# mkofler96/DeepSDF

Measured on AMD Instinct MI355X. Metric: SDF point-samples/sec per training step (8x512 decoder, 16384 pts), higher is better.
Workload: dtype f32; 1 GPU; configs[1]: 64 synthetic sphere-SDF scenes, latent_dim=256, 8x512 decoder + layer-4 skip, weight-norm, dropout 0.2, 16384 pts/step (64 scenes x 256 samples), fp32; headline_config=True, parallelism=dp1

## Files before the change

### deepsdf_amd/csrc/dsdf_api.hip

```cpp
#include "../../include/dsdf.h"

#include <hip/hip_runtime.h>
#include <math.h>
#include <stdarg.h>
#include <stdio.h>
#include <string.h>

#include <stdlib.h>

#include <algorithm>
#include <atomic>
#ifdef DSDF_LAB
#include <vector>
#endif

#include "dwstream.hpp"
#include "sample.hpp"
#include "fused.hpp"
#include "fused_bf16x8.hpp"
#include "gemm.hpp"
#include "kernels.hpp"
#include "mcubes.hpp"
#include "meshsdf.hpp"
#include "msgrid.hpp"
// ... 534 lines not shown
struct FamilyKernels {
  FwdKernel fwd; int fwd_block;
  FwdKernel fwd_act;
  BwdKernel bwd;
  FwdBwdKernel fwd_bwd;
  DwKernel dw;
  int block;
};
const FamilyKernels KERNELS[FAM_COUNT] = {
     {nullptr, 0, nullptr, nullptr, nullptr, nullptr, 0},
     {fused_forward_kernel, 256, fused_forward_kernel, fused_backward_kernel, fused_fwd_bwd_kernel, dw_stream_kernel, 256},
     {fused_forward_split_kernel, 256, fused_forward_split_kernel, fused_backward_split_kernel, fused_fwd_bwd_split_kernel,
                          dw_stream_split_kernel, 256},
     {fused_forward_bf16x8_kernel, F8_THREADS, fused_forward_bf16_kernel, fused_backward_kernel, fused_fwd_bf16_bwd_kernel,
                          dw_stream_kernel, 256},
     {fused_forward_bf16x8_kernel, F8_THREADS, fused_forward_bf16_kernel, fused_backward_split_kernel,
                          fused_fwd_bf16_bwd_split_kernel, dw_stream_split_kernel, 256},
     {fused_forward_h32_kernel, 256, fused_forward_h32_kernel, nullptr, fused_fwd_bwd_h32_kernel, dw_stream_kernel, 256},
     {fused_forward_n128_kernel, 256, fused_forward_n128_kernel, fused_backward_kernel, fused_fwd_bwd_n128_kernel,
                          dw_stream_kernel, 256},
     {nullptr, 0, nullptr, nullptr, fused_fwd_bwd_w32_kernel, dw_stream_kernel, 64},
     {nullptr, 0, nullptr, nullptr, fused_fwd_bwd_w32x2_kernel, dw_stream_kernel, 64},
};

bool fused_eligible(const DsdfNet* net) {
  if (net_variant(net)) return false;
  if (net->in_dim[0] > FMAXW) return false;
  for (int l = 0; l < net->n_layers - 1; ++l)
    if (net->in_dim[l] > FMAXW || net->out_dim[l] > FMAXW) return false;
  return net->in_dim[net->n_layers - 1] <= FMAXW;
}

Path pick_path(const DsdfNet* net, int64_t n, Entry entry, const Switches& sw) {
  Path p{FAM_LAYERED, FROWS, false, false};
  if (sw.no_fused || !fused_eligible(net)) return p;
  p.fused = true;
  p.merged = entry == ENTRY_TRAIN && !sw.no_merge;
  if (net->fwd_bf16 || net->gemm_split) {
    p.family = !net->fwd_bf16 ? FAM_SPLIT : (net->gemm_split ? FAM_BF16_SPLIT : FAM_BF16);
    return p;
  }
  int wmax = 0;
  for (int l = 0; l < net->n_layers; ++l) {
    wmax = std::max(wmax, net->in_dim[l]);
    if (l < net->n_layers - 1) wmax = std::max(wmax, net->out_dim[l]);
  }
  const bool narrow = !sw.no_narrow && wmax <= 128;
  p.family = narrow ? FAM_N128 : FAM_FP32;
  const bool rows32 = entry == ENTRY_INFER || p.merged;
  if (!rows32 || sw.frows64 || n <= 0) return p;
  if (p.merged && narrow && !sw.no_w32 && (wmax <= FWW || (wmax <= FWW2 && !sw.no_w32x2))) {
    p.family = wmax <= FWW ? FAM_W32 : FAM_W32X2;
    p.frows = 32;
  } else if (n <= 32ll * (chip_waves() / 4)) {
    p.family = FAM_H32;
    p.frows = 32;
  }
  return p;
}

struct Drop { bool on; uint32_t thr; float scale; };
Drop drop_of(const DsdfNet* net, int layer, int training) {
  Drop d{training && ((net->dropout_mask >> layer) & 1) && net->dropout_p > 0.f, 0u, 1.0f};
  if (d.on) {
    d.thr = (uint32_t)std::min(lround((double)net->dropout_p * 65536.0), 65535l);
    d.scale = 1.0f / (1.0f - net->dropout_p);
  }
  return d;
}
float mask_scale_of(const DsdfNet* net, int layer, int training) { return drop_of(net, layer, training).scale; }

struct Call {
  const DsdfNet* net;
  Switches sw;
  Path path;
  Plan P;
  DsdfParamLayout L;
  Packed pk;
  void* ws;
  const float* packed;
  const float* params;
  int64_t n;
  hipStream_t st;
  int training;
  const uint32_t* keys;
  uint32_t row_offset;
  template <typename T>
  T* at(size_t off) const { return reinterpret_cast<T*>(static_cast<char*>(ws) + off); }
};

int run_gather(const Call& c, const float* table, const DsdfBatch* b, const float* input, int64_t ld_in) {
  GatherArgs g;
  memset(&g, 0, sizeof(g));
  g.table = table; g.L = c.net->latent_size; g.G = c.net->geom_dim;
  if (b) { g.xyz = b->xyz; g.seg_scene = b->seg_scene; g.seg_offset = b->seg_offset; g.R = (int)b->n_segments; }
  g.input = input; g.ld_in = ld_in; g.n = (int)c.n;
  const int W0 = c.net->latent_size + c.net->geom_dim;
  const bool drop = c.net->latent_dropout && c.training && c.keys != nullptr && c.net->latent_size > 0;
  if (drop) { g.drop_key = c.keys[LATENT_DROPOUT_KEY]; g.drop_thr = latent_drop_thr(); g.drop_scale = 1.0f / (1.0f - LATENT_DROPOUT_P); g.row_offset = c.row_offset; }
  g.ndst = 0;
  g.dst[g.ndst++] = GatherDst{c.at<float>(c.P.in_off[0]), c.P.ld_in[0], 0, 0, W0, drop ? 1 : 0};
  for (int l = 1; l < c.net->n_layers; ++l) {
    if ((c.net->skip_mask >> l) & 1) g.dst[g.ndst++] = GatherDst{c.at<float>(c.P.in_off[l]), c.P.ld_in[l], c.net->out_dim[l - 1], 0, W0, 0};
    else if (c.net->xyz_in_all) g.dst[g.ndst++] = GatherDst{c.at<float>(c.P.in_off[l]), c.P.ld_in[l], c.net->out_dim[l - 1], c.net->latent_size, c.net->geom_dim, 0};
  }
  hipLaunchKernelGGL(gather_concat_kernel, dim3((unsigned)((c.n + 3) / 4)), dim3(256), 0, c.st, g);
  LAUNCH_OK("gather_concat_kernel");
  return 0;
}

#ifdef DSDF_LAB
struct LabStamps { const char* env; size_t bytes; bool zero; unsigned long long* dev; };
struct LabScope {
  LabStamps& s;
  LabScope(LabStamps& site, hipStream_t st) : s(site) {
    if (!s.dev && getenv(s.env)) (void)hipMalloc(&s.dev, s.bytes);
    if (s.dev && s.zero) (void)hipMemsetAsync(s.dev, 0, s.bytes, st);
  }
  ~LabScope() {
    if (!s.dev || !getenv(s.env)) return;
    (void)hipDeviceSynchronize();
    std::vector<unsigned long long> h(s.bytes / 8);
    (void)hipMemcpy(h.data(), s.dev, s.bytes, hipMemcpyDeviceToHost);
    FILE* f = fopen(getenv(s.env), "wb");
    if (f) { fwrite(h.data(), 1, s.bytes, f); fclose(f); }
  }
};
#endif

struct HoistRenorm { float max_norm; float* dlat; long long nzero; };
int run_hoist(const Call& c, const float* table, const DsdfBatch* b, FusedSeg* seg, const HoistRenorm* renorm = nullptr) {
  if (c.net->latent_size < 1 || c.net->latent_size > HOIST_MAXL)
    return fail(DSDF_E_INVALID, "segment mode needs 1 <= latent_size <= %d (got %d)", HOIST_MAXL, c.net->latent_size);
  const int ks = skip_layer(c.net);
  HoistArgs h;
  memset(&h, 0, sizeof(h));
  memset(seg, 0, sizeof(*seg));
  h.nh = ks > 0 ? 2 : 1;
  h.W[0] = c.packed + c.pk.w_off[0]; h.ldw[0] = c.pk.ldw[0]; h.c0[0] = 0; h.out[0] = c.net->out_dim[0];
  seg->h[0].layer = 0; seg->h[0].wx = h.W[0] + c.net->latent_size; seg->h[0].ldw = c.pk.ldw[0];
  seg->h[1].layer = -1;
  if (ks > 0) {
    h.W[1] = c.packed + c.pk.w_off[ks]; h.ldw[1] = c.pk.ldw[ks]; h.c0[1] = c.net->out_dim[ks - 1]; h.out[1] = c.net->out_dim[ks];
    seg->h[1].layer = ks; seg->h[1].wx = h.W[1] + h.c0[1] + c.net->latent_size; seg->h[1].ldw = c.pk.ldw[ks];
  }
  h.L = c.net->latent_size; h.seg_scene = b->seg_scene; h.table = table; h.R = (int)b->n_segments;
  h.U = c.at<float>(c.P.hoistU_off); h.ldu = c.P.ldu;
  h.bf16 = c.net->fwd_bf16 ? 1 : 0;
  if (renorm != nullptr) {
    h.max_norm = renorm->max_norm; h.zr = c.at<float>(c.P.zr_off);
    h.dlat = renorm->nzero > 0 ? renorm->dlat : nullptr; h.nzero = renorm->nzero;
  }
  const int rows = h.out[0] + (ks > 0 ? h.out[1] : 0);
  const dim3 hgrid((unsigned)((rows + 3) / 4), (unsigned)((h.R + HOIST_SC - 1) / HOIST_SC));
  switch ((h.L + 63) >> 6) {
    case 1: hipLaunchKernelGGL(seg_hoist_kernel<1>, hgrid, dim3(256), 0, c.st, h); break;
    case 2: hipLaunchKernelGGL(seg_hoist_kernel<2>, hgrid, dim3(256), 0, c.st, h); break;
    case 3: case 4: hipLaunchKernelGGL(seg_hoist_kernel<4>, hgrid, dim3(256), 0, c.st, h); break;
    default: hipLaunchKernelGGL(seg_hoist_kernel<8>, hgrid, dim3(256), 0, c.st, h); break;
  }
  LAUNCH_OK("seg_hoist_kernel");
  seg->wg_per_seg = (int)(b->seg_len / c.P.frows);
  seg->xyz = b->xyz; seg->G = c.net->geom_dim; seg->U = h.U; seg->ldu = h.ldu;
  return 0;
}

int run_fused_forward(const Call& c, bool store_act, float* y_out, float* u_out, const FusedSeg* seg = nullptr,
                      FusedFwdArgs* defer = nullptr) {
  const int last = c.net->n_layers - 1;
  FusedFwdArgs a;
  memset(&a, 0, sizeof(a));
  a.n_hidden = last; a.N = (int)c.n; a.W0 = c.net->in_dim[0];
  a.x0 = c.at<float>(c.P.in_off[0]); a.ldx0 = c.P.ld_in[0];
  a.row_offset = c.row_offset;
  for (int l = 0; l < last; ++l) {
    FusedLayer& y = a.ly[l];
    y.wf = c.net->fwd_bf16 ? c.packed + c.pk.wfb_off[l] : (c.net->gemm_split ? c.packed + c.pk.ws_off[l] : c.packed + c.pk.wf_off[l]);
    y.wplane = (int)(c.pk.ws_plane[l] * 2);
    y.wf32 = c.packed + c.pk.wf_off[l];
    y.bias = c.params + c.L.bias_off[l];
    y.out = store_act ? c.at<float>(c.P.in_off[l + 1]) : nullptr;
    y.ld_out = c.P.ld_in[l + 1];
    y.in = c.net->in_dim[l]; y.out_dim = c.net->out_dim[l]; y.U = c.pk.uf[l];
    const Drop drop = drop_of(c.net, l, c.training);
    if (drop.on) { y.drop_thr = drop.thr; y.drop_key = c.keys[l]; y.drop_scale = drop.scale; }
    y.x0_col = ((c.net->skip_mask >> (l + 1)) & 1) ? c.net->out_dim[l] : -1;
    y.maskbits = store_act ? c.at<uint32_t>(c.P.mask_off[l]) : nullptr;
    if (seg != nullptr) {
      y.x0_col = -1;
      if (l == 0) y.in = 0;
      else if ((c.net->skip_mask >> l) & 1) y.in = c.net->out_dim[l - 1];
    }
  }
  if (seg != nullptr) a.seg = *seg;
  a.w_last = c.packed + c.pk.w_off[last]; a.b_last = c.params + c.L.bias_off[last]; a.in_last = c.net->in_dim[last];
  a.use_tanh = c.net->use_tanh; a.y_out = y_out; a.u_out = u_out;
  if (defer != nullptr) {
    a.ly[last - 1].out = nullptr;
    *defer = a;
    return 0;
  }
  double wmac = 0;
  for (int l = 0; l < last; ++l) wmac += (double)c.net->in_dim[l] * c.net->out_dim[l];
  ProfScope ps(DSDF_PROF_FUSED_FWD, 2.0 * (double)c.n * wmac, c.st);
#ifdef DSDF_LAB
  static LabStamps stamps{"DSDF_LAB_DBG", 8192 * 64 * 8, false, nullptr};
  LabScope lab(stamps, c.st);
  a.dbg = stamps.dev;
#endif
  const FamilyKernels& k = KERNELS[c.path.family];
  const FwdKernel kernel = store_act ? k.fwd_act : k.fwd;
  if (kernel == nullptr) return fail(DSDF_E_LAUNCH, "internal: kernel family %d has no forward of its own", (int)c.path.family);
  const dim3 grid((unsigned)((c.n + c.P.frows - 1) / c.P.frows));
  hipLaunchKernelGGL(kernel, grid, dim3(store_act ? k.block : k.fwd_block), 0, c.st, a);
  LAUNCH_OK("fused_forward_kernel");
  return 0;
}

int run_hidden_forward(const Call& c, bool save_ln = true) {
  for (int l = 0; l < c.net->n_layers - 1; ++l) {
    NtArgs a;
    memset(&a, 0, sizeof(a));
    a.A = c.at<float>(c.P.in_off[l]); a.lda = c.P.ld_in[l];
    a.B = c.packed + c.pk.w_off[l]; a.ldb = c.pk.ldw[l];
    a.C = c.at<float>(c.P.in_off[l + 1]); a.ldc = c.P.ld_in[l + 1];
    a.M = (int)c.n; a.N = c.net->out_dim[l]; a.K = c.net->in_dim[l];
    a.bias = c.params + c.L.bias_off[l];
    a.relu = 1;
    const Drop drop = drop_of(c.net, l, c.training);
    if (ln_applied(c.net, l)) {
      a.C = c.at<float>(c.P.lnx_off[l]);
      TRY(launch_nt<EPI_PLAIN>(a, c.st));
      LnFwdArgs f;
      memset(&f, 0, sizeof(f));
      f.y = a.C; f.ldy = a.ldc; f.gamma = c.params + c.L.ln_w_off[l]; f.beta = c.params + c.L.ln_b_off[l];
      f.out = c.at<float>(c.P.in_off[l + 1]); f.ldo = c.P.ld_in[l + 1]; f.n = (int)c.n; f.width = c.net->out_dim[l];
      f.save = save_ln ? 1 : 0; f.rstd = save_ln ? c.at<float>(c.P.lnr_off[l]) : nullptr;
      if (drop.on) { f.drop_thr = drop.thr; f.drop_key = c.keys[l]; f.drop_scale = drop.scale; f.row_offset = c.row_offset; }
      hipLaunchKernelGGL(ln_fwd_kernel, dim3((unsigned)((c.n + 3) / 4)), dim3(256), 0, c.st, f);
      LAUNCH_OK("ln_fwd_kernel");
      continue;
    }
    if (drop.on) { a.drop_thr = drop.thr; a.drop_key = c.keys[l]; a.drop_scale = drop.scale; a.row_offset = c.row_offset; }
    TRY(launch_nt<EPI_FWD>(a, c.st));
  }
  return 0;
}

struct FuseAdam { const DsdfAdamCfg* cfg; float* params; float* exp_avg; float* exp_avg_sq; float* packed; bool used; };

struct FinSrc { const float* slabs; int nsplit; long long slab; int ldc; const float* colsum; int npart; int ldcs; };
struct GradSink { float* grads; int accumulate; const FuseAdam* fz; };
FinArgs fin_args(const Call& c, int l, const FinSrc& src, const GradSink& to) {
  FinArgs f;
  memset(&f, 0, sizeof(f));
  f.slabs = src.slabs; f.nsplit = src.nsplit; f.slab = src.slab; f.ldc = src.ldc;
  f.colsum = src.colsum; f.npart = src.npart; f.ldcs = src.ldcs;
  f.g = c.L.g_off[l] >= 0 ? c.params + c.L.g_off[l] : nullptr;
  f.v = c.params + c.L.v_off[l];
  f.dg = c.L.g_off[l] >= 0 ? to.grads + c.L.g_off[l] : nullptr;
  f.dv = to.grads + c.L.v_off[l];
  f.db = to.grads + c.L.bias_off[l];
  f.out = c.net->out_dim[l]; f.in = c.net->in_dim[l]; f.accumulate = to.accumulate;
  if (to.fz != nullptr) {
    const DsdfAdamCfg* ad = to.fz->cfg;
    const double bc1 = 1.0 - pow((double)ad->beta1, (double)ad->step), bc2 = 1.0 - pow((double)ad->beta2, (double)ad->step);
    f.adam = 1;
    f.pb = to.fz->params + c.L.bias_off[l]; f.mb = to.fz->exp_avg + c.L.bias_off[l]; f.sb = to.fz->exp_avg_sq + c.L.bias_off[l];
    f.pv = to.fz->params + c.L.v_off[l];    f.mv = to.fz->exp_avg + c.L.v_off[l];    f.sv = to.fz->exp_avg_sq + c.L.v_off[l];
    if (c.L.g_off[l] >= 0) { f.pg = to.fz->params + c.L.g_off[l]; f.mg = to.fz->exp_avg + c.L.g_off[l]; f.sg = to.fz->exp_avg_sq + c.L.g_off[l]; }
    int r0 = 0;
    for (int q = 0; q < l; ++q) r0 += c.net->out_dim[q];
    f.scale_out = to.fz->packed + c.pk.scale_off + r0;
    f.omb1 = 1.0f - ad->beta1; f.b2 = ad->beta2; f.omb2 = 1.0f - ad->beta2;
    f.step_size = (float)((double)ad->lr_decoder / bc1); f.bc2_sqrt = (float)sqrt(bc2); f.eps = ad->eps;
  }
  return f;
}

int add_dz_to_input(const Call& c, bool used_dzB, float* d_input, int64_t ld_din) {
  const long long tot = (long long)c.n * c.P.W0;
  hipLaunchKernelGGL(add2_kernel, dim3((unsigned)((tot + 255) / 256)), dim3(256), 0, c.st, c.at<float>(c.P.dzA_off), c.P.ldz,
                     used_dzB ? c.at<float>(c.P.dzB_off) : nullptr, c.P.ldz, d_input, (long long)ld_din, (int)c.n, c.P.W0);
  LAUNCH_OK("add2_kernel");
  return 0;
}

LastArgs last_args(const Call& c, bool backward = false) {
  const int last = c.net->n_layers - 1;
  LastArgs a;
  memset(&a, 0, sizeof(a));
  a.a = c.at<float>(c.P.in_off[last]); a.lda = c.P.ld_in[last]; a.in = c.net->in_dim[last];
  a.w = c.packed + c.pk.w_off[last]; a.b = c.params + c.L.bias_off[last]; a.n = (int)c.n; a.use_tanh = c.net->use_tanh;
  if (!backward) return a;
  a.dp_prev = c.at<float>(c.P.dp_off[0]);
  a.lddp = c.P.ld_dp; a.mask_scale = mask_scale_of(c.net, last - 1, c.training);
  a.part_dw = c.at<float>(c.P.part_off); a.ld_part = c.P.ld_part;
  a.part_colsum = c.at<float>(c.P.part_off) + c.P.ld_in[last];
  a.part_db = c.at<float>(c.P.partdb_off); a.part_loss = c.at<float>(c.P.partloss_off);
  a.n_act = c.net->out_dim[last - 1];
  return a;
}

int run_backward(const Call& c, const GradSink& to, int ncols_dz, bool* used_dzB, bool want_dw, bool* xyz_acc = nullptr) {
  const int last = c.net->n_layers - 1;
  if (want_dw) {
    const int w = c.P.ld_part;
// ... 2469 lines not shown
```

### deepsdf_amd/csrc/kernels.hpp

```cpp
#pragma once
#include "common.hpp"

namespace dsdf {

constexpr int FSEG_MAXW = 512;

__global__ void latent_renorm_kernel(float* __restrict__ table, int L, const int64_t* __restrict__ seg_scene,
                                     int R, float max_norm, float* __restrict__ dlat, long long nzero) {
  if (dlat != nullptr)
    for (long long i = ((long long)blockIdx.x * blockDim.x + threadIdx.x) * 4; i < nzero; i += (long long)gridDim.x * blockDim.x * 4) {
      if (i + 3 < nzero) *reinterpret_cast<float4*>(dlat + i) = make_float4(0.f, 0.f, 0.f, 0.f);
      else for (long long q = i; q < nzero; ++q) dlat[q] = 0.f;
    }
  const int r = blockIdx.x * (blockDim.x >> 6) + (threadIdx.x >> 6);
  const int lane = threadIdx.x & 63;
  if (r >= R || max_norm <= 0.f) return;
  const int64_t j = seg_scene[r];
  int dup = 0;
  for (int q = lane; q < r; q += 64) dup |= (seg_scene[q] == j);
  if (__any(dup)) return;
  float* row = table + (size_t)j * L;
  float ss = 0.f;
  for (int c = lane; c < L; c += 64) { const float v = row[c]; ss += v * v; }
  ss = wave_sum(ss);
  const float nu = sqrtf(ss);
  if (nu > max_norm) {
    const float s = max_norm / (nu + 1e-7f);
    for (int c = lane; c < L; c += 64) row[c] *= s;
  }
}

struct GatherDst { float* ptr; int ld; int col0; int src0; int ncols; int drop; };
struct GatherArgs {
  const float* table; int L; const float* xyz; int G;
  const int64_t* seg_scene; const int64_t* seg_offset; int R;
  const float* input; long long ld_in;
  uint32_t drop_key, drop_thr; float drop_scale; uint32_t row_offset;
  int n; int ndst; GatherDst dst[DSDF_MAX_LAYERS + 1];
};
__global__ void gather_concat_kernel(const GatherArgs p) {
  const int n = blockIdx.x * (blockDim.x >> 6) + (threadIdx.x >> 6);
  const int lane = threadIdx.x & 63;
  if (n >= p.n) return;
  const int W = p.L + p.G;
  const float* src_lat;
  const float* src_xyz;
  if (p.input != nullptr) {
    src_lat = p.input + (size_t)n * p.ld_in;
    src_xyz = src_lat + p.L;
  } else {
    int lo = 0, hi = p.R;
    while (hi - lo > 1) { const int mid = (lo + hi) >> 1; if (p.seg_offset[mid] <= n) lo = mid; else hi = mid; }
    src_lat = p.table + (size_t)p.seg_scene[lo] * p.L;
    src_xyz = p.xyz + (size_t)n * p.G;
  }
  const uint32_t g = p.row_offset + (uint32_t)n;
  for (int c = lane; c < W; c += 64) {
    const float v = c < p.L ? src_lat[c] : src_xyz[c - p.L];
    for (int d = 0; d < p.ndst; ++d) {
      const GatherDst& D = p.dst[d];
      if (c < D.src0 || c >= D.src0 + D.ncols) continue;
      float o = v;
      if (D.drop && c < p.L) o = drop_keep(drop_pair_hash(drop_col_key((uint32_t)c, p.drop_key), g), g, p.drop_thr) ? v * p.drop_scale : 0.f;
      D.ptr[(size_t)n * D.ld + D.col0 + (c - D.src0)] = o;
    }
  }
}

__global__ void latent_drop_bwd_kernel(float* dz, int ld, int n, int L, uint32_t key, uint32_t thr, float scale, uint32_t row_offset) {
  const long long i = (long long)blockIdx.x * blockDim.x + threadIdx.x;
  if (i >= (long long)n * L) return;
  const int r = (int)(i / L), c = (int)(i % L);
  const uint32_t g = row_offset + (uint32_t)r;
  float* q = dz + (size_t)r * ld + c;
  *q = drop_keep(drop_pair_hash(drop_col_key((uint32_t)c, key), g), g, thr) ? *q * scale : 0.f;
}

__global__ void acc_cols_kernel(const float* src, int lds, float* dst, int ldd, int c0, int n, int w, int accumulate) {
  const long long i = (long long)blockIdx.x * blockDim.x + threadIdx.x;
  if (i >= (long long)n * w) return;
  const int r = (int)(i / w), j = (int)(i % w);
  float* q = dst + (size_t)r * ldd + c0 + j;
  const float v = src[(size_t)r * lds + j];
  *q = accumulate ? *q + v : v;
}

__global__ void last_xyz_grad_kernel(const float* d_sdf, const float* u_in, const float* w_xyz, int G, int use_tanh, float* dst,
                                     int ldd, int c0, int n, int accumulate) {
  const long long i = (long long)blockIdx.x * blockDim.x + threadIdx.x;
  if (i >= (long long)n * G) return;
  const int r = (int)(i / G), j = (int)(i % G);
  const float u = u_in[r];
  const float t1 = use_tanh ? tanhf(u) : u;
  const float y = tanhf(t1);
  float du = d_sdf[r] * (1.f - y * y);
  if (use_tanh) du *= (1.f - t1 * t1);
  float* q = dst + (size_t)r * ldd + c0 + j;
  const float v = du * w_xyz[j];
  *q = accumulate ? *q + v : v;
}

constexpr int HOIST_MAXL = 512;
constexpr int HOIST_SC = 16;
struct HoistArgs {
  int nh;
  const float* W[2]; int ldw[2]; int c0[2]; int out[2];
  int L; const int64_t* seg_scene; const float* table; int R;
  float* U; int ldu;
  int bf16;
  float max_norm;
  float* zr;
  float* dlat; long long nzero;
};
template <int KU>
__device__ __forceinline__ void seg_hoist_body(const HoistArgs& p, const int n, const int t) {
  const int lane = threadIdx.x & 63;
  const int s0 = blockIdx.y * HOIST_SC;
  const long long myscene = (long long)p.seg_scene[min(s0 + (lane & (HOIST_SC - 1)), p.R - 1)];
  const float* wrow = p.W[t] + (size_t)n * p.ldw[t] + p.c0[t];
  float wv[KU], v[HOIST_SC][KU];
#pragma unroll
  for (int k = 0; k < KU; ++k) wv[k] = wrow[min(lane + 64 * k, p.L - 1)];
#pragma unroll
  for (int q = 0; q < HOIST_SC; ++q) {
    const float* row = p.table + (size_t)__shfl(myscene, q, 64) * p.L;
#pragma unroll
    for (int k = 0; k < KU; ++k) v[q][k] = row[min(lane + 64 * k, p.L - 1)];
  }
#pragma unroll
  for (int k = 0; k < KU; ++k) {
    const bool ok = lane + 64 * k < p.L;
    wv[k] = ok ? wv[k] : 0.f;
#pragma unroll
    for (int q = 0; q < HOIST_SC; ++q) v[q][k] = ok ? v[q][k] : 0.f;
  }
  static_assert(HOIST_SC == 16, "wave_sum16");
  if (p.max_norm > 0.f) {
    float ss[HOIST_SC];
#pragma unroll
    for (int q = 0; q < HOIST_SC; ++q) {
      ss[q] = 0.f;
#pragma unroll
      for (int k = 0; k < KU; ++k) ss[q] += v[q][k] * v[q][k];
    }
    const float mine = wave_sum16(ss, lane);
#pragma unroll
    for (int q = 0; q < HOIST_SC; ++q) {
      const float nu = sqrtf(__shfl(mine, wave_sum16_lane(q), 64));
      if (nu > p.max_norm) {
        const float sc = p.max_norm / (nu + 1e-7f);
#pragma unroll
        for (int k = 0; k < KU; ++k) v[q][k] *= sc;
      }
    }
  }
  if (p.zr != nullptr && blockIdx.x == 0 && threadIdx.x < 64) {
#pragma unroll
    for (int q = 0; q < HOIST_SC; ++q)
      if (s0 + q < p.R)
#pragma unroll
        for (int k = 0; k < KU; ++k)
          if (lane + 64 * k < p.L) p.zr[(size_t)(s0 + q) * p.L + lane + 64 * k] = v[q][k];
  }
  float a[HOIST_SC];
#pragma unroll
  for (int q = 0; q < HOIST_SC; ++q) a[q] = 0.f;
#pragma unroll
  for (int k = 0; k < KU; ++k) {
    const float w = p.bf16 ? (float)(__bf16)wv[k] : wv[k];
#pragma unroll
    for (int q = 0; q < HOIST_SC; ++q) {
      const float x = p.bf16 ? (float)(__bf16)v[q][k] : v[q][k];
      if (lane + 64 * k < p.L) a[q] = fmaf(w, x, a[q]);
    }
  }
  const float r = wave_sum16(a, lane);
  const int qi = wave_sum16_index(lane);
  if ((lane & 3) == 0 && s0 + qi < p.R) p.U[((size_t)(s0 + qi) * 2 + t) * p.ldu + n] = r;
}
template <int KU>
__global__ __launch_bounds__(256) void seg_hoist_kernel(const HoistArgs p) {
  if (p.dlat != nullptr) {
    const long long nb = (long long)gridDim.x * gridDim.y, b = (long long)blockIdx.y * gridDim.x + blockIdx.x;
    for (long long i = (b * 256 + threadIdx.x) * 4; i < p.nzero; i += nb * 256 * 4) {
      if (i + 3 < p.nzero) *reinterpret_cast<float4*>(p.dlat + i) = make_float4(0.f, 0.f, 0.f, 0.f);
      else for (long long q = i; q < p.nzero; ++q) p.dlat[q] = 0.f;
    }
  }
  int n = blockIdx.x * 4 + (threadIdx.x >> 6);
  int t = 0;
  if (n >= p.out[0]) { n -= p.out[0]; t = 1; }
  if (t >= p.nh || n >= p.out[t]) return;
  seg_hoist_body<KU>(p, n, t);
}

constexpr int SDW_ROWS_RIDE = 32, SDW_ROWS_WIDE = 8;
constexpr int SDW_LDS_FLOATS = 64 * SDW_ROWS_RIDE + 256 * 4 + 2 * 64;
struct SegDwArgs {
  int nh; const float* cs[2]; const float* xsum[2]; int out[2];
  int ldcs, nwg, wg_per_seg, R, L, G;
  const int64_t* seg_scene; const float* table;
  const float* zr;
  float* HS; int ldh; long long hstride;
};
template <int SDW_ROWS>
__device__ __forceinline__ void seg_dw_body(const SegDwArgs& p, int bidx, float* lds) {
  constexpr int SDW_SLOTS = 256 / SDW_ROWS;
  float (*css)[SDW_ROWS] = reinterpret_cast<float (*)[SDW_ROWS]>(lds);
  float (*xred)[SDW_ROWS][4] = reinterpret_cast<float (*)[SDW_ROWS][4]>(lds + 64 * SDW_ROWS);
  long long* srow = reinterpret_cast<long long*>(lds + 64 * SDW_ROWS + SDW_SLOTS * SDW_ROWS * 4);
  const int tid = threadIdx.x;
  int blk = bidx, t = 0;
  const int b0 = (p.out[0] + SDW_ROWS - 1) / SDW_ROWS;
  if (blk >= b0) { blk -= b0; t = 1; }
  const int i0 = blk * SDW_ROWS;
  const float* cs = p.cs[t];
  const int r_ld = tid & (SDW_ROWS - 1), s_ld = tid / SDW_ROWS;
  const bool rok = i0 + r_ld < p.out[t];
  const int ird = min(i0 + r_ld, p.out[t] - 1);
  float xa[4] = {0.f, 0.f, 0.f, 0.f};
  for (int wg0 = s_ld; wg0 < p.nwg; wg0 += 8 * SDW_SLOTS) {
    float tx[8][4];
#pragma unroll
    for (int u = 0; u < 8; ++u) {
      const int wg = wg0 + u * SDW_SLOTS;
#pragma unroll
      for (int j = 0; j < 4; ++j)
        tx[u][j] = p.xsum[t][((size_t)min(wg, p.nwg - 1) * 4 + j) * p.ldcs + ird];
    }
#pragma unroll
    for (int u = 0; u < 8; ++u)
#pragma unroll
      for (int j = 0; j < 4; ++j) xa[j] += (rok && wg0 + u * SDW_SLOTS < p.nwg && j < p.G) ? tx[u][j] : 0.f;
  }
  constexpr int NC = HOIST_MAXL / 256;
  float acc[NC][SDW_ROWS];
#pragma unroll
  for (int k = 0; k < NC; ++k)
#pragma unroll
    for (int r = 0; r < SDW_ROWS; ++r) acc[k][r] = 0.f;
  for (int s0 = 0; s0 < p.R; s0 += 64) {
    __syncthreads();
    if (p.wg_per_seg <= 16) {
#pragma unroll
      for (int q = 0; q < 64 / SDW_SLOTS; ++q) {
        const int sl = s_ld + SDW_SLOTS * q, sg = s0 + sl;
        float tg[16];
#pragma unroll
        for (int g = 0; g < 16; ++g)
          tg[g] = cs[(size_t)(min(sg, p.R - 1) * p.wg_per_seg + min(g, p.wg_per_seg - 1)) * p.ldcs + ird];
        float a = 0.f;
#pragma unroll
        for (int g = 0; g < 16; ++g) a += (sg < p.R && rok && g < p.wg_per_seg) ? tg[g] : 0.f;
        css[sl][r_ld] = a;
      }
    } else {
      for (int sl = 0; sl < 64; ++sl) {
        const int sg = s0 + sl;
        float a = 0.f;
        if (sg < p.R && rok)
          for (int g0 = s_ld; g0 < p.wg_per_seg; g0 += 8 * SDW_SLOTS) {
            float tg[8];
#pragma unroll
            for (int u = 0; u < 8; ++u) {
              const int g = g0 + u * SDW_SLOTS;
              tg[u] = g < p.wg_per_seg ? cs[(size_t)(sg * p.wg_per_seg + g) * p.ldcs + i0 + r_ld] : 0.f;
            }
#pragma unroll
            for (int u = 0; u < 8; ++u) a += tg[u];
          }
        xred[s_ld][r_ld][0] = a;
        __syncthreads();
        if (tid < SDW_ROWS) {
          float v = 0.f;
#pragma unroll
          for (int q = 0; q < SDW_SLOTS; ++q) v += xred[q][tid][0];
          css[sl][tid] = v;
        }
        __syncthreads();
        if (sg + 1 >= p.R) {
          for (int z = sl + 1 + s_ld; z < 64; z += SDW_SLOTS) css[z][r_ld] = 0.f;
          break;
        }
      }
    }
    if (tid < 64) {
      const int sg = min(s0 + tid, p.R - 1);
      srow[tid] = p.zr != nullptr ? (long long)sg * p.L : (long long)p.seg_scene[sg] * p.L;
    }
    __syncthreads();
    const float* lat = p.zr != nullptr ? p.zr : p.table;
#pragma unroll
    for (int k = 0; k < NC; ++k) {
      const int c = tid + 256 * k;
      if (c < p.L) {
        float v[64];
#pragma unroll
        for (int u = 0; u < 64; ++u) v[u] = lat[srow[u] + c];
#pragma unroll
        for (int u = 0; u < 64; ++u) {
          const float4* cq = reinterpret_cast<const float4*>(css[u]);
#pragma unroll
          for (int r4 = 0; r4 < SDW_ROWS / 4; ++r4) {
            const float4 cv = cq[r4];
            acc[k][4 * r4 + 0] = fmaf(cv.x, v[u], acc[k][4 * r4 + 0]);
            acc[k][4 * r4 + 1] = fmaf(cv.y, v[u], acc[k][4 * r4 + 1]);
            acc[k][4 * r4 + 2] = fmaf(cv.z, v[u], acc[k][4 * r4 + 2]);
            acc[k][4 * r4 + 3] = fmaf(cv.w, v[u], acc[k][4 * r4 + 3]);
          }
        }
      }
    }
  }
  float* hs = p.HS + (size_t)t * p.hstride;
#pragma unroll
  for (int k = 0; k < NC; ++k) {
    const int c = tid + 256 * k;
    if (c < p.L)
#pragma unroll
      for (int r = 0; r < SDW_ROWS; ++r)
        if (i0 + r < p.out[t]) hs[(size_t)(i0 + r) * p.ldh + c] = acc[k][r];
  }
  __syncthreads();
#pragma unroll
  for (int j = 0; j < 4; ++j) xred[s_ld][r_ld][j] = xa[j];
  __syncthreads();
  if (tid < SDW_ROWS * 4) {
    const int r = tid >> 2, j = tid & 3;
    if (j < p.G && i0 + r < p.out[t]) {
      float v = 0.f;
#pragma unroll
      for (int q = 0; q < SDW_SLOTS; ++q) v += xred[q][r][j];
      hs[(size_t)(i0 + r) * p.ldh + p.L + j] = v;
    }
  }
}

struct WnLayer {
  const float* v; const float* g; float* W; float* WT; int out, in, ldw, ldwt; int row0; int tile0; int tcols;
  float* Wf; float* WTf;
  __bf16* Wfb;
  int Uf, UTf;
  __bf16* Ws; __bf16* WTs;
  long long ws_plane, wts_plane;
};
struct AdamRide {
// ... 1102 lines not shown
```

Measured before the change: 13.33 million point-samples/s.

## Share renormed latents across waves via LDS and compute two weight rows per wave

Restructures the segment hoist kernel so each wave loads and renormalizes only four latent rows, then shares all sixteen through shared memory. Each wave now handles two weight rows instead of one, which halves the grid in x and removes the per-wave redundant latent loads and norm reductions. It also adds a narrower 4-way wave reduction for the norms. The cost is a __syncthreads, extra LDS traffic, and higher register pressure from holding two weight rows.

```diff
diff --git a/deepsdf_amd/csrc/dsdf_api.hip b/deepsdf_amd/csrc/dsdf_api.hip
--- a/deepsdf_amd/csrc/dsdf_api.hip
+++ b/deepsdf_amd/csrc/dsdf_api.hip
@@ -710,7 +710,7 @@
     h.dlat = renorm->nzero > 0 ? renorm->dlat : nullptr; h.nzero = renorm->nzero;
   }
   const int rows = h.out[0] + (ks > 0 ? h.out[1] : 0);
-  const dim3 hgrid((unsigned)((rows + 3) / 4), (unsigned)((h.R + HOIST_SC - 1) / HOIST_SC));
+  const dim3 hgrid((unsigned)((rows + HOIST_ROWS - 1) / HOIST_ROWS), (unsigned)((h.R + HOIST_SC - 1) / HOIST_SC));
   switch ((h.L + 63) >> 6) {
     case 1: hipLaunchKernelGGL(seg_hoist_kernel<1>, hgrid, dim3(256), 0, c.st, h); break;
     case 2: hipLaunchKernelGGL(seg_hoist_kernel<2>, hgrid, dim3(256), 0, c.st, h); break;
diff --git a/deepsdf_amd/csrc/kernels.hpp b/deepsdf_amd/csrc/kernels.hpp
--- a/deepsdf_amd/csrc/kernels.hpp
+++ b/deepsdf_amd/csrc/kernels.hpp
@@ -112,74 +112,48 @@
   float* zr;
   float* dlat; long long nzero;
 };
+constexpr int HOIST_ROWS = 8;
+constexpr int HOIST_RPW = HOIST_ROWS / 4;
+__device__ __forceinline__ constexpr int wave_sum4_lane(int j) { return 32 * ((j >> 1) & 1) + 16 * (j & 1); }
+__device__ __forceinline__ float wave_sum4(const float (&a)[4], int lane) {
+  float b2[2];
+  const bool h5 = lane & 32, h4 = lane & 16;
+#pragma unroll
+  for (int j = 0; j < 2; ++j) b2[j] = (h5 ? a[2 + j] : a[j]) + __shfl_xor(h5 ? a[j] : a[2 + j], 32, 64);
+  float r = (h4 ? b2[1] : b2[0]) + __shfl_xor(h4 ? b2[0] : b2[1], 16, 64);
+  r += __shfl_xor(r, 8, 64);
+  r += __shfl_xor(r, 4, 64);
+  r += __shfl_xor(r, 2, 64);
+  r += __shfl_xor(r, 1, 64);
+  return r;
+}
 template <int KU>
-__device__ __forceinline__ void seg_hoist_body(const HoistArgs& p, const int n, const int t) {
-  const int lane = threadIdx.x & 63;
+__global__ __launch_bounds__(256) void seg_hoist_kernel(const HoistArgs p) {
+  static_assert(HOIST_SC == 16 && HOIST_ROWS % 4 == 0, "wave_sum16; four segments and HOIST_RPW weight rows per wave");
+  __shared__ float zs[HOIST_SC][64 * KU];
+  const int lane = threadIdx.x & 63, wave = threadIdx.x >> 6;
   const int s0 = blockIdx.y * HOIST_SC;
   const long long myscene = (long long)p.seg_scene[min(s0 + (lane & (HOIST_SC - 1)), p.R - 1)];
-  const float* wrow = p.W[t] + (size_t)n * p.ldw[t] + p.c0[t];
-  float wv[KU], v[HOIST_SC][KU];
-#pragma unroll
-  for (int k = 0; k < KU; ++k) wv[k] = wrow[min(lane + 64 * k, p.L - 1)];
-#pragma unroll
-  for (int q = 0; q < HOIST_SC; ++q) {
-    const float* row = p.table + (size_t)__shfl(myscene, q, 64) * p.L;
-#pragma unroll
-    for (int k = 0; k < KU; ++k) v[q][k] = row[min(lane + 64 * k, p.L - 1)];
-  }
-#pragma unroll
-  for (int k = 0; k < KU; ++k) {
-    const bool ok = lane + 64 * k < p.L;
-    wv[k] = ok ? wv[k] : 0.f;
-#pragma unroll
-    for (int q = 0; q < HOIST_SC; ++q) v[q][k] = ok ? v[q][k] : 0.f;
-  }
-  static_assert(HOIST_SC == 16, "wave_sum16");
-  if (p.max_norm > 0.f) {
-    float ss[HOIST_SC];
-#pragma unroll
-    for (int q = 0; q < HOIST_SC; ++q) {
-      ss[q] = 0.f;
-#pragma unroll
-      for (int k = 0; k < KU; ++k) ss[q] += v[q][k] * v[q][k];
-    }
-    const float mine = wave_sum16(ss, lane);
-#pragma unroll
-    for (int q = 0; q < HOIST_SC; ++q) {
-      const float nu = sqrtf(__shfl(mine, wave_sum16_lane(q), 64));
-      if (nu > p.max_norm) {
-        const float sc = p.max_norm / (nu + 1e-7f);
-#pragma unroll
-        for (int k = 0; k < KU; ++k) v[q][k] *= sc;
-      }
-    }
-  }
-  if (p.zr != nullptr && blockIdx.x == 0 && threadIdx.x < 64) {
-#pragma unroll
-    for (int q = 0; q < HOIST_SC; ++q)
-      if (s0 + q < p.R)
-#pragma unroll
-        for (int k = 0; k < KU; ++k)
-          if (lane + 64 * k < p.L) p.zr[(size_t)(s0 + q) * p.L + lane + 64 * k] = v[q][k];
-  }
-  float a[HOIST_SC];
-#pragma unroll
-  for (int q = 0; q < HOIST_SC; ++q) a[q] = 0.f;
-#pragma unroll
-  for (int k = 0; k < KU; ++k) {
-    const float w = p.bf16 ? (float)(__bf16)wv[k] : wv[k];
-#pragma unroll
-    for (int q = 0; q < HOIST_SC; ++q) {
-      const float x = p.bf16 ? (float)(__bf16)v[q][k] : v[q][k];
-      if (lane + 64 * k < p.L) a[q] = fmaf(w, x, a[q]);
-    }
-  }
-  const float r = wave_sum16(a, lane);
-  const int qi = wave_sum16_index(lane);
-  if ((lane & 3) == 0 && s0 + qi < p.R) p.U[((size_t)(s0 + qi) * 2 + t) * p.ldu + n] = r;
-}
-template <int KU>
-__global__ __launch_bounds__(256) void seg_hoist_kernel(const HoistArgs p) {
+  int wn[HOIST_RPW], wt[HOIST_RPW]; bool wok[HOIST_RPW];
+  float wv[HOIST_RPW][KU];
+#pragma unroll
+  for (int j = 0; j < HOIST_RPW; ++j) {
+    int n = blockIdx.x * HOIST_ROWS + wave * HOIST_RPW + j, t = 0;
+    if (n >= p.out[0]) { n -= p.out[0]; t = 1; }
+    wok[j] = t < p.nh && n < p.out[t];
+    if (!wok[j]) { n = 0; t = 0; }
+    wn[j] = n; wt[j] = t;
+    const float* wrow = p.W[t] + (size_t)n * p.ldw[t] + p.c0[t];
+#pragma unroll
+    for (int k = 0; k < KU; ++k) wv[j][k] = wrow[min(lane + 64 * k, p.L - 1)];
+  }
+  float z[4][KU];
+#pragma unroll
+  for (int j = 0; j < 4; ++j) {
+    const float* row = p.table + (size_t)__shfl(myscene, 4 * wave + j, 64) * p.L;
+#pragma unroll
+    for (int k = 0; k < KU; ++k) z[j][k] = row[min(lane + 64 * k, p.L - 1)];
+  }
   if (p.dlat != nullptr) {
     const long long nb = (long long)gridDim.x * gridDim.y, b = (long long)blockIdx.y * gridDim.x + blockIdx.x;
     for (long long i = (b * 256 + threadIdx.x) * 4; i < p.nzero; i += nb * 256 * 4) {
@@ -187,11 +161,66 @@
       else for (long long q = i; q < p.nzero; ++q) p.dlat[q] = 0.f;
     }
   }
-  int n = blockIdx.x * 4 + (threadIdx.x >> 6);
-  int t = 0;
-  if (n >= p.out[0]) { n -= p.out[0]; t = 1; }
-  if (t >= p.nh || n >= p.out[t]) return;
-  seg_hoist_body<KU>(p, n, t);
+#pragma unroll
+  for (int k = 0; k < KU; ++k) {
+    const bool ok = lane + 64 * k < p.L;
+#pragma unroll
+    for (int j = 0; j < 4; ++j) z[j][k] = ok ? z[j][k] : 0.f;
+  }
+  if (p.max_norm > 0.f) {
+    float ss[4];
+#pragma unroll
+    for (int j = 0; j < 4; ++j) {
+      ss[j] = 0.f;
+#pragma unroll
+      for (int k = 0; k < KU; ++k) ss[j] += z[j][k] * z[j][k];
+    }
+    const float mine = wave_sum4(ss, lane);
+#pragma unroll
+    for (int j = 0; j < 4; ++j) {
+      const float nu = sqrtf(__shfl(mine, wave_sum4_lane(j), 64));
+      if (nu > p.max_norm) {
+        const float sc = p.max_norm / (nu + 1e-7f);
+#pragma unroll
+        for (int k = 0; k < KU; ++k) z[j][k] *= sc;
+      }
+    }
+  }
+#pragma unroll
+  for (int j = 0; j < 4; ++j) {
+    const int q = 4 * wave + j;
+#pragma unroll
+    for (int k = 0; k < KU; ++k) zs[q][lane + 64 * k] = z[j][k];
+    if (p.zr != nullptr && blockIdx.x == 0 && s0 + q < p.R)
+#pragma unroll
+      for (int k = 0; k < KU; ++k)
+        if (lane + 64 * k < p.L) p.zr[(size_t)(s0 + q) * p.L + lane + 64 * k] = z[j][k];
+  }
+  __syncthreads();
+  float v[HOIST_SC][KU];
+#pragma unroll
+  for (int q = 0; q < HOIST_SC; ++q)
+#pragma unroll
+    for (int k = 0; k < KU; ++k) v[q][k] = zs[q][lane + 64 * k];
+#pragma unroll
+  for (int j = 0; j < HOIST_RPW; ++j) {
+    float a[HOIST_SC];
+#pragma unroll
+    for (int q = 0; q < HOIST_SC; ++q) a[q] = 0.f;
+#pragma unroll
+    for (int k = 0; k < KU; ++k) {
+      const float w0 = lane + 64 * k < p.L ? wv[j][k] : 0.f;
+      const float w = p.bf16 ? (float)(__bf16)w0 : w0;
+#pragma unroll
+      for (int q = 0; q < HOIST_SC; ++q) {
+        const float x = p.bf16 ? (float)(__bf16)v[q][k] : v[q][k];
+        if (lane + 64 * k < p.L) a[q] = fmaf(w, x, a[q]);
+      }
+    }
+    const float r = wave_sum16(a, lane);
+    const int qi = wave_sum16_index(lane);
+    if (wok[j] && (lane & 3) == 0 && s0 + qi < p.R) p.U[((size_t)(s0 + qi) * 2 + wt[j]) * p.ldu + wn[j]] = r;
+  }
 }
 
 constexpr int SDW_ROWS_RIDE = 32, SDW_ROWS_WIDE = 8;
```

Result: no change. 13.38 million point-samples/s (median of 6 runs) (+0.4%).
